# cvlab-epfl/gecco

Measured on NVIDIA B200. Metric: point clouds/sec (2048 pts, full EDM sampler), higher is better.
Workload: dtype bf16

## Files before the change

gecco_b200/csrc/attention_pool_tc.cu:

```cuda
#include "common.cuh"
#include "kernels.cuh"
#include "ptx.cuh"

namespace gecco {
namespace {

constexpr int TM = 128;
constexpr int NI = 64;
constexpr int HD = 48;
constexpr int NH = 8;
constexpr int NP = NH / 2;
constexpr int C = NH * HD;
constexpr int SLOTS = 4;
constexpr int WIN_BYTES = TM * 128;
constexpr int Q_BYTES = 2 * NI * 128;
constexpr int P_BYTES = 2 * TM * 128;
constexpr int TMEM_COLS = 512;
constexpr int THREADS = 128 + 256;
constexpr int SMEM_BYTES = 1024  + 2 * Q_BYTES + 2 * SLOTS * WIN_BYTES + 2 * P_BYTES + 256 ;
static_assert(SMEM_BYTES <= 232448, "shared memory budget");

__host__ __device__ constexpr uint32_t umma_idesc_bf16_bmn(int M, int N) { return umma_idesc_bf16(M, N) | (1u << 16); }
__device__ __forceinline__ uint64_t umma_desc_mn_sw128(uint32_t saddr, uint32_t lbo_bytes) {
  uint64_t d = 0;
  d |= static_cast<uint64_t>((saddr & 0x3FFFFu) >> 4);
  d |= static_cast<uint64_t>(lbo_bytes >> 4) << 16;
  d |= static_cast<uint64_t>(1024 >> 4) << 32;
  d |= static_cast<uint64_t>(1) << 46;
  d |= static_cast<uint64_t>(2) << 61;
  return d;
}

struct PParams {
  const __nv_bfloat16* q_ind;
  int clouds, rows_per_cloud, valid_rows;
  int tiles, splits, tps;
  int items;
  float* partial;
  __nv_bfloat16* out;
  long long ldo;
};

struct Cursor {
  int item, item_stride, items;
  int tile, tile_end;
  int cloud, pair, split;
  __device__ __forceinline__ void open(const PParams& p) {
    if (item >= items) return;
    split = item % p.splits;
    pair = (item / p.splits) % NP;
    cloud = item / (p.splits * NP);
    tile = split * p.tps;
    tile_end = min(p.tiles, tile + p.tps);
  }
  __device__ __forceinline__ void init(const PParams& p, int first, int stride) {
// ... 15 lines not shown
  float y;
  asm("ex2.approx.ftz.f32 %0, %1;" : "=f"(y) : "f"(x));
  return y;
}
__device__ __forceinline__ void tmem_ld32(uint32_t addr, uint32_t (&r)[32]) {
  asm volatile(
      "tcgen05.ld.sync.aligned.32x32b.x32.b32 {%0,%1,%2,%3,%4,%5,%6,%7,%8,%9,%10,%11,%12,%13,%14,%15,%16,%17,%18,%19,%20,"
      "%21,%22,%23,%24,%25,%26,%27,%28,%29,%30,%31}, [%32];"
      : "=r"(r[0]), "=r"(r[1]), "=r"(r[2]), "=r"(r[3]), "=r"(r[4]), "=r"(r[5]), "=r"(r[6]), "=r"(r[7]), "=r"(r[8]),
        "=r"(r[9]), "=r"(r[10]), "=r"(r[11]), "=r"(r[12]), "=r"(r[13]), "=r"(r[14]), "=r"(r[15]), "=r"(r[16]),
        "=r"(r[17]), "=r"(r[18]), "=r"(r[19]), "=r"(r[20]), "=r"(r[21]), "=r"(r[22]), "=r"(r[23]), "=r"(r[24]),
        "=r"(r[25]), "=r"(r[26]), "=r"(r[27]), "=r"(r[28]), "=r"(r[29]), "=r"(r[30]), "=r"(r[31])
      : "r"(addr)
      : "memory");
}
__device__ __forceinline__ void sts128(uint32_t addr, uint32_t a, uint32_t b, uint32_t c, uint32_t d) {
  asm volatile("st.shared.v4.b32 [%0], {%1,%2,%3,%4};" ::"r"(addr), "r"(a), "r"(b), "r"(c), "r"(d) : "memory");
}

__global__ void __launch_bounds__(THREADS, 1)
pool_tc_kernel(const __grid_constant__ CUtensorMap tma_k, const __grid_constant__ CUtensorMap tma_v, const PParams p) {
  extern __shared__ uint8_t smem_raw[];
  uint8_t* smem = reinterpret_cast<uint8_t*>((reinterpret_cast<uintptr_t>(smem_raw) + 1023) & ~uintptr_t(1023));
  uint8_t* sQ = smem;
  uint8_t* sK = sQ + 2 * Q_BYTES;
  uint8_t* sV = sK + SLOTS * WIN_BYTES;
  uint8_t* sP = sV + SLOTS * WIN_BYTES;
  uint64_t* bars = reinterpret_cast<uint64_t*>(sP + 2 * P_BYTES);
  uint64_t* k_full = bars;
  uint64_t* k_empty = k_full + SLOTS;
  uint64_t* v_full = k_empty + SLOTS;
  uint64_t* v_empty = v_full + SLOTS;
  uint64_t* q_ready = v_empty + SLOTS;
  uint64_t* s_full = q_ready + 2;
  uint64_t* p_full = s_full + 2;
  uint64_t* o_full = p_full + 2;
  uint64_t* o_read = o_full + 2;
  uint32_t* tmem_slot = reinterpret_cast<uint32_t*>(o_read + 2);

  const int warp = threadIdx.x >> 5;
  const int uwarp = uniform_warp_idx();
  const int lane = threadIdx.x & 31;

  if (warp == 0 && lane == 0) {
    tma_prefetch_desc(&tma_k);
    tma_prefetch_desc(&tma_v);
  }
  if (warp == 1 && lane == 0) {
    for (int i = 0; i < SLOTS; ++i) {
      mbar_init(&k_full[i], 1);
      mbar_init(&k_empty[i], 1);
      mbar_init(&v_full[i], 1);
      mbar_init(&v_empty[i], 1);
    }
    for (int i = 0; i < 2; ++i) {
      mbar_init(&q_ready[i], 4);
      mbar_init(&s_full[i], 1);
      mbar_init(&p_full[i], 4);
      mbar_init(&o_full[i], 1);
      mbar_init(&o_read[i], 4);
    }
    fence_barrier_init();
  }
  if (warp == 2) tmem_alloc<TMEM_COLS>(tmem_slot);
  tc_fence_before_sync();
  __syncthreads();
  tc_fence_after_sync();
  const uint32_t tmem_base = *tmem_slot;
  pdl_wait();
  pdl_launch_dependents();

  Cursor cur[2];
  cur[0].init(p, blockIdx.x * 2 + 0, gridDim.x * 2);
  cur[1].init(p, blockIdx.x * 2 + 1, gridDim.x * 2);

  if (warp == 0 && lane == 0) {
    uint32_t gk = 0, gv = 0;
    while (!cur[0].done() || !cur[1].done()) {
#pragma unroll
      for (int kind = 0; kind < 2; ++kind) {
#pragma unroll
        for (int w = 0; w < 2; ++w) {
          if (cur[w].done()) continue;
          const int row = cur[w].cloud * p.rows_per_cloud + cur[w].tile * TM;
          for (int j = 0; j < 2; ++j) {
            const int col = kind == 0 ? (2 * cur[w].pair + j) * HD : cur[w].pair * 2 * HD + j * 64;
            if (kind == 0) {
              const uint32_t slot = gk % SLOTS, use = gk / SLOTS;
              mbar_wait(&k_empty[slot], (use & 1u) ^ 1u);
              mbar_arrive_expect_tx(&k_full[slot], WIN_BYTES);
              tma_load_2d(sK + slot * WIN_BYTES, &tma_k, &k_full[slot], col, row);
              ++gk;
            } else {
              const uint32_t slot = gv % SLOTS, use = gv / SLOTS;
              mbar_wait(&v_empty[slot], (use & 1u) ^ 1u);
              mbar_arrive_expect_tx(&v_full[slot], WIN_BYTES);
              tma_load_2d(sV + slot * WIN_BYTES, &tma_v, &v_full[slot], col, row);
              ++gv;
            }
          }
        }
      }
#pragma unroll
      for (int w = 0; w < 2; ++w)
        if (!cur[w].done()) cur[w].next(p);
    }
  } else if (uwarp == 1) {
    constexpr uint32_t idesc_s = umma_idesc_bf16(TM, TM);
    constexpr uint32_t idesc_o = umma_idesc_bf16_bmn(TM, 2 * HD);
    const uint32_t sQ_u = uniform_u32(smem_u32(sQ)), sK_u = uniform_u32(smem_u32(sK)), sV_u = uniform_u32(smem_u32(sV));
    const uint32_t sP_u = uniform_u32(smem_u32(sP));
    const uint32_t tmem_u = uniform_u32(tmem_base);
    uint32_t gk = 0, gv = 0;
    uint32_t nS[2] = {0, 0};
    uint32_t nO[2] = {0, 0};
    uint32_t nQ[2] = {0, 0};
    int pend[2] = {0, 0};
    auto issue_s = [&](int w) {
      if (nS[w] > 0) mbar_wait(&o_read[w], (nS[w] - 1) & 1u);
      if (cur[w].first_of_item(p)) {
        mbar_wait(&q_ready[w], nQ[w] & 1u);
        ++nQ[w];
      }
      const uint32_t k0 = gk % SLOTS, k1 = (gk + 1) % SLOTS;
      mbar_wait(&k_full[k0], (gk / SLOTS) & 1u);
      mbar_wait(&k_full[k1], ((gk + 1) / SLOTS) & 1u);
      tc_fence_after_sync();
      if (elect_one()) {
        const uint32_t qa = sQ_u + w * Q_BYTES;
#pragma unroll
        for (int hh = 0; hh < 2; ++hh) {
          const uint32_t kb = sK_u + (hh ? k1 : k0) * WIN_BYTES;
#pragma unroll
          for (int kk = 0; kk < HD / 16; ++kk)
            umma_bf16_ss(tmem_u + w * 256 + hh * 128, umma_desc_k_sw128(qa) + 2 * kk, umma_desc_k_sw128(kb) + 2 * kk, idesc_s,
                         kk ? 1u : 0u);
        }
        umma_commit(&k_empty[k0]);
        umma_commit(&k_empty[k1]);
        umma_commit(&s_full[w]);
      }
      __syncwarp();
      gk += 2;
      ++nS[w];
      pend[w] = 1;
      cur[w].next(p);
    };
    auto issue_o = [&](int w) {
      mbar_wait(&p_full[w], nO[w] & 1u);
      const uint32_t v0 = gv % SLOTS, v1 = (gv + 1) % SLOTS;
      mbar_wait(&v_full[v0], (gv / SLOTS) & 1u);
      mbar_wait(&v_full[v1], ((gv + 1) / SLOTS) & 1u);
      tc_fence_after_sync();
      if (elect_one()) {
        const uint32_t vb = sV_u + v0 * WIN_BYTES;
#pragma unroll
        for (int kk = 0; kk < TM / 16; ++kk) {
          const uint64_t da = umma_desc_k_sw128(sP_u + w * P_BYTES + (kk >> 2) * (TM * 128)) + 2 * (kk & 3);
          const uint64_t db = umma_desc_mn_sw128(vb + kk * 2048, WIN_BYTES);
          umma_bf16_ss(tmem_u + w * 256, da, db, idesc_o, kk ? 1u : 0u);
        }
        umma_commit(&v_empty[v0]);
        umma_commit(&v_empty[v1]);
        umma_commit(&o_full[w]);
      }
      __syncwarp();
      gv += 2;
      ++nO[w];
      pend[w] = 0;
    };
#pragma unroll
    for (int w = 0; w < 2; ++w)
      if (!cur[w].done()) issue_s(w);
    while (pend[0] || pend[1]) {
#pragma unroll
      for (int w = 0; w < 2; ++w)
        if (pend[w]) issue_o(w);
#pragma unroll
      for (int w = 0; w < 2; ++w)
        if (!cur[w].done()) issue_s(w);
    }
  } else if (warp >= 4) {
    const int w = (warp - 4) >> 2;
    const int q = warp & 3;
    const uint32_t row = q * 32 + lane;
    const uint32_t x7 = (row & 7u) << 4;
    const uint32_t t_addr = tmem_base + (static_cast<uint32_t>(q * 32) << 16) + w * 256 + (q >> 1) * 128;
    const uint32_t o_addr = tmem_base + (static_cast<uint32_t>(q * 32) << 16) + w * 256 + (q >> 1) * HD;
    const uint32_t p_row = smem_u32(sP) + w * P_BYTES + row * 128u;
    Cursor& c = cur[w];
    uint32_t n = 0;
    float m = -INFINITY, l = 0.f;
    float acc[HD];
#pragma unroll
    for (int d = 0; d < HD; ++d) acc[d] = 0.f;

    while (!c.done()) {
      if (c.first_of_item(p)) {
        const int t = threadIdx.x - 128 - w * 128;
        for (int i = t; i < 2 * NI * (HD / 8); i += 128) {
          const int r = i / (HD / 8), ch = i - r * (HD / 8);
          const uint4 v = __ldg(reinterpret_cast<const uint4*>(p.q_ind + ((long long)c.pair * 2 * NI + r) * HD + ch * 8));
          *reinterpret_cast<uint4*>(sQ + w * Q_BYTES + r * 128 + ((ch ^ (r & 7)) << 4)) = v;
        }
        fence_proxy_async_smem();
        __syncwarp();
        if (lane == 0) mbar_arrive(&q_ready[w]);
      }
      const int nvalid = p.valid_rows - c.tile * TM;
      mbar_wait(&s_full[w], n & 1u);
      tc_fence_after_sync();
      float mref = m;
      if (c.first_of_item(p)) {
        float mx = -INFINITY;
#pragma unroll 1
        for (int cb = 0; cb < TM; cb += 32) {
          uint32_t s[32];
          tmem_ld32(t_addr + cb, s);
          tmem_ld_wait();
          if (nvalid >= cb + 32) {
#pragma unroll
            for (int i = 0; i < 32; ++i) mx = fmaxf(mx, __uint_as_float(s[i]));
          } else {
#pragma unroll
            for (int i = 0; i < 32; ++i) mx = fmaxf(mx, cb + i < nvalid ? __uint_as_float(s[i]) : -INFINITY);
          }
        }
        mref = mx;
        m = mx;
      }
      float sum, umax;
      for (;;) {
        sum = 0.f;
        umax = -INFINITY;
#pragma unroll 1
        for (int cb = 0; cb < TM; cb += 32) {
          uint32_t s[32];
          tmem_ld32(t_addr + cb, s);
          tmem_ld_wait();
          uint32_t pk[16];
          if (nvalid >= cb + 32) {
#pragma unroll
            for (int i = 0; i < 16; ++i) {
              const float s0 = __uint_as_float(s[2 * i]), s1 = __uint_as_float(s[2 * i + 1]);
              umax = fmaxf(umax, fmaxf(s0, s1));
              const float a = ex2f(s0 - mref), b = ex2f(s1 - mref);
              sum += a + b;
              pk[i] = pack_bf16x2(a, b);
            }
          } else {
#pragma unroll
            for (int i = 0; i < 16; ++i) {
              const bool v0 = cb + 2 * i < nvalid, v1 = cb + 2 * i + 1 < nvalid;
              const float s0 = v0 ? __uint_as_float(s[2 * i]) : -INFINITY, s1 = v1 ? __uint_as_float(s[2 * i + 1]) : -INFINITY;
              umax = fmaxf(umax, fmaxf(s0, s1));
              const float a = ex2f(s0 - mref), b = ex2f(s1 - mref);
              sum += a + b;
              pk[i] = pack_bf16x2(a, b);
            }
          }
          const uint32_t kb_row = p_row + (cb >> 6) * (TM * 128);
          const uint32_t ch0 = (cb & 32) >> 3;
#pragma unroll
          for (int i = 0; i < 4; ++i)
            sts128(kb_row + (((ch0 + i) << 4) ^ x7), pk[4 * i], pk[4 * i + 1], pk[4 * i + 2], pk[4 * i + 3]);
        }
        if (!__any_sync(0xffffffffu, umax > mref + 64.f)) break;
        if (umax > mref) {
          const float r = ex2f(mref - umax);
          l *= r;
#pragma unroll
          for (int d = 0; d < HD; ++d) acc[d] *= r;
          mref = umax;
          m = umax;
        }
      }
      l += sum;
      fence_proxy_async_smem();
      tc_fence_before_sync();
      __syncwarp();
      if (lane == 0) mbar_arrive(&p_full[w]);
      mbar_wait(&o_full[w], n & 1u);
      tc_fence_after_sync();
      {
        uint32_t o[HD];
        tmem_ld16(o_addr, o);
        tmem_ld16(o_addr + 16, o + 16);
        tmem_ld16(o_addr + 32, o + 32);
        tmem_ld_wait();
        tc_fence_before_sync();
        __syncwarp();
        if (lane == 0) mbar_arrive(&o_read[w]);
#pragma unroll
        for (int d = 0; d < HD; ++d) acc[d] += __uint_as_float(o[d]);
      }
      if (umax > m) {
        const float r = ex2f(m - umax);
        l *= r;
#pragma unroll
        for (int d = 0; d < HD; ++d) acc[d] *= r;
        m = umax;
      }
      ++n;
      if (c.last_of_item()) {
        const int head = 2 * c.pair + (row >> 6), ind = row & 63;
        if (p.splits == 1) {
          const float inv = 1.0f / l;
          uint4* dst = reinterpret_cast<uint4*>(p.out + ((long long)c.cloud * NI + ind) * p.ldo + head * HD);
#pragma unroll
          for (int i = 0; i < HD / 8; ++i)
            dst[i] = make_uint4(pack_bf16x2(acc[8 * i + 0] * inv, acc[8 * i + 1] * inv), pack_bf16x2(acc[8 * i + 2] * inv, acc[8 * i + 3] * inv),
                                pack_bf16x2(acc[8 * i + 4] * inv, acc[8 * i + 5] * inv), pack_bf16x2(acc[8 * i + 6] * inv, acc[8 * i + 7] * inv));
        } else {
          float* dst = p.partial + ((((long long)c.cloud * NH + head) * p.splits + c.split) * NI + ind) * (HD + 2);
#pragma unroll
          for (int d = 0; d < HD; d += 2) *reinterpret_cast<float2*>(dst + d) = make_float2(acc[d], acc[d + 1]);
          *reinterpret_cast<float2*>(dst + HD) = make_float2(m, l);
        }
        m = -INFINITY;
        l = 0.f;
#pragma unroll
        for (int d = 0; d < HD; ++d) acc[d] = 0.f;
      }
      c.next(p);
    }
  }

  tc_fence_before_sync();
  __syncthreads();
  if (warp == 2) {
    tc_fence_after_sync();
    tmem_dealloc<TMEM_COLS>(tmem_base);
  }
}

}

bool pool_tc_supported(const gecco_pool_args& a) {
  return a.heads == NH && a.head_dim == HD && a.inducers == NI && a.rows_per_cloud % TM == 0 && a.ld % 8 == 0 &&
// ... 13 lines not shown
  PParams p;
  p.q_ind = static_cast<const __nv_bfloat16*>(a.q_inducers);
  p.clouds = a.clouds; p.rows_per_cloud = a.rows_per_cloud; p.valid_rows = a.valid_rows;
  p.tiles = ceil_div(a.valid_rows, TM);
  const int sms = sm_count();
  int splits = (2 * sms) / (a.clouds * NP);
  if (splits > a.splits) splits = a.splits;
  if (splits > p.tiles) splits = p.tiles;
  if (splits < 1 || a.partial == nullptr) splits = 1;
  p.tps = ceil_div(p.tiles, splits);
  p.splits = ceil_div(p.tiles, p.tps);
  p.items = a.clouds * NP * p.splits;
  p.partial = a.partial;
  p.out = static_cast<__nv_bfloat16*>(a.out_bf16);
  p.ldo = a.ldo;
  *splits_used = p.splits;
  int grid = ceil_div(p.items, 2);
  if (grid > sms) grid = sms;

  static bool attr_set = false;
  if (!attr_set) {
    cudaError_t e = cudaFuncSetAttribute(pool_tc_kernel, cudaFuncAttributeMaxDynamicSharedMemorySize, SMEM_BYTES);
    if (e != cudaSuccess) return fail_cuda(e, "cudaFuncSetAttribute(pool_tc_kernel)");
    attr_set = true;
  }
  cudaLaunchConfig_t cfg = {};
  cfg.gridDim = dim3(grid);
  cfg.blockDim = dim3(THREADS);
  cfg.dynamicSmemBytes = SMEM_BYTES;
  cfg.stream = stream;
// ... 13 lines not shown
```

gecco_b200/csrc/attention_tc.cu:

```cuda
#include "common.cuh"
#include "kernels.cuh"
#include "ptx.cuh"

namespace gecco {
namespace {

constexpr int TM = 128;
constexpr int NI = 64;
constexpr int HD = 48;
constexpr int NH = 8;
constexpr int C = NH * HD;
constexpr int BK = 64;
constexpr int NKB = C / BK;
constexpr int QSLOTS = 4;
constexpr int Q_SLOT_BYTES = TM * BK * 2;
constexpr int K_KB_BYTES = NI * BK * 2;
constexpr int VT_BYTES = C * NI * 2;
constexpr int P_BYTES = TM * NI * 2;
constexpr int Y_BYTES = TM * HD * 2;
constexpr int O_COLS = C;
constexpr int TMEM_COLS = 512;
constexpr int THREADS = 128 + 256;
constexpr int SMEM_BYTES = 1024  + QSLOTS * Q_SLOT_BYTES + NKB * K_KB_BYTES + VT_BYTES + 2 * P_BYTES + 2 * Y_BYTES +
                           256 ;
static_assert(SMEM_BYTES <= 232448, "shared memory budget");

struct UParams {
  int tiles_per_cloud, num_tiles, tiles_per_cta;
};

__device__ __forceinline__ float ex2f(float x) {
  float y;
  asm("ex2.approx.ftz.f32 %0, %1;" : "=f"(y) : "f"(x));
  return y;
}
__device__ __forceinline__ void tmem_ld32(uint32_t addr, uint32_t (&r)[32]) {
  asm volatile(
      "tcgen05.ld.sync.aligned.32x32b.x32.b32 {%0,%1,%2,%3,%4,%5,%6,%7,%8,%9,%10,%11,%12,%13,%14,%15,%16,%17,%18,%19,%20,"
// ... 5 lines not shown
      : "r"(addr)
      : "memory");
}
__device__ __forceinline__ void sts128(uint32_t addr, uint32_t a, uint32_t b, uint32_t c, uint32_t d) {
  asm volatile("st.shared.v4.b32 [%0], {%1,%2,%3,%4};" ::"r"(addr), "r"(a), "r"(b), "r"(c), "r"(d) : "memory");
}

__global__ void __launch_bounds__(THREADS, 1)
unpool_tc_kernel(const __grid_constant__ CUtensorMap tma_q, const __grid_constant__ CUtensorMap tma_k,
                 const __grid_constant__ CUtensorMap tma_vt, const __grid_constant__ CUtensorMap tma_y, const UParams p) {
  extern __shared__ uint8_t smem_raw[];
  uint8_t* smem = reinterpret_cast<uint8_t*>((reinterpret_cast<uintptr_t>(smem_raw) + 1023) & ~uintptr_t(1023));
  uint8_t* sQ = smem;
  uint8_t* sK = sQ + QSLOTS * Q_SLOT_BYTES;
  uint8_t* sVT = sK + NKB * K_KB_BYTES;
  uint8_t* sP = sVT + VT_BYTES;
  uint8_t* sY = sP + 2 * P_BYTES;
  uint64_t* bars = reinterpret_cast<uint64_t*>(sY + 2 * Y_BYTES);
  uint64_t* q_full = bars;
  uint64_t* q_empty = q_full + QSLOTS;
  uint64_t* kv_full = q_empty + QSLOTS;
  uint64_t* s_full = kv_full + 1;
  uint64_t* p_full = s_full + 2;
  uint64_t* pv_done = p_full + 2;
  uint64_t* tile_done = pv_done + 2;
  uint32_t* tmem_slot = reinterpret_cast<uint32_t*>(tile_done + 1);

  const int warp = threadIdx.x >> 5;
  const int uwarp = uniform_warp_idx();
  const int lane = threadIdx.x & 31;
  const int tile_begin = blockIdx.x * p.tiles_per_cta;
  const int tile_end = min(tile_begin + p.tiles_per_cta, p.num_tiles);

  if (warp == 0 && lane == 0) {
    tma_prefetch_desc(&tma_q);
    tma_prefetch_desc(&tma_k);
    tma_prefetch_desc(&tma_vt);
    tma_prefetch_desc(&tma_y);
  }
  if (warp == 1 && lane == 0) {
    for (int i = 0; i < QSLOTS; ++i) {
      mbar_init(&q_full[i], 1);
      mbar_init(&q_empty[i], 1);
    }
    mbar_init(kv_full, 1);
    mbar_init(tile_done, 1);
    for (int i = 0; i < 2; ++i) {
      mbar_init(&s_full[i], 1);
      mbar_init(&p_full[i], 4);
      mbar_init(&pv_done[i], 1);
    }
    fence_barrier_init();
  }
  if (warp == 2) tmem_alloc<TMEM_COLS>(tmem_slot);
  tc_fence_before_sync();
  __syncthreads();
  tc_fence_after_sync();
  const uint32_t tmem_base = *tmem_slot;
  pdl_wait();
  pdl_launch_dependents();

  if (warp == 0 && lane == 0) {
    int cloud_loaded = -1;
    uint32_t it = 0, g = 0;
    for (int t = tile_begin; t < tile_end; ++t, ++it) {
// ... 5 lines not shown
        tma_load_2d(sVT, &tma_vt, kv_full, 0, cloud * C);
        tma_load_2d(sVT + VT_BYTES / 2, &tma_vt, kv_full, 0, cloud * C + C / 2);
        cloud_loaded = cloud;
      }
      for (int h = 0; h < NH; ++h, ++g) {
        const uint32_t slot = g % QSLOTS, use = g / QSLOTS;
        mbar_wait(&q_empty[slot], (use & 1u) ^ 1u);
        mbar_arrive_expect_tx(&q_full[slot], Q_SLOT_BYTES);
        tma_load_2d(sQ + slot * Q_SLOT_BYTES, &tma_q, &q_full[slot], h * HD, t * TM);
      }
    }
  } else if (uwarp == 1) {
    constexpr uint32_t idesc_s = umma_idesc_bf16(TM, NI);
    constexpr uint32_t idesc_o = umma_idesc_bf16(TM, HD);
    const uint32_t sQ_u = uniform_u32(smem_u32(sQ)), sK_u = uniform_u32(smem_u32(sK));
    const uint32_t sVT_u = uniform_u32(smem_u32(sVT)), sP_u = uniform_u32(smem_u32(sP));
    const uint32_t tmem_u = uniform_u32(tmem_base);
    int cloud_loaded = -1;
    uint32_t it = 0, ncl = 0, gs = 0;
    auto issue_s = [&](int h) {
      const uint32_t slot = gs % QSLOTS, use = gs / QSLOTS;
      mbar_wait(&q_full[slot], use & 1u);
      tc_fence_after_sync();
      if (elect_one()) {
#pragma unroll
        for (int kk = 0; kk < HD / 16; ++kk) {
          const int col = h * HD + kk * 16;
          const uint64_t da = umma_desc_k_sw128(sQ_u + slot * Q_SLOT_BYTES) + 2 * kk;
          const uint64_t db = umma_desc_k_sw128(sK_u + (col / BK) * K_KB_BYTES) + (((col % BK) * 2) >> 4);
          umma_bf16_ss(tmem_u + O_COLS + (h & 1) * NI, da, db, idesc_s, kk ? 1u : 0u);
        }
// ... 8 lines not shown
      if (cloud != cloud_loaded) {
        mbar_wait(kv_full, ncl & 1u);
        tc_fence_after_sync();
        cloud_loaded = cloud;
        ++ncl;
      }
      issue_s(0);
      issue_s(1);
      for (int h = 0; h < NH; ++h) {
        const uint32_t w = h & 1u, use = it * (NH / 2) + (h >> 1);
        mbar_wait(&p_full[w], use & 1u);
        tc_fence_after_sync();
        if (elect_one()) {
#pragma unroll
          for (int kk = 0; kk < NI / 16; ++kk) {
            const uint64_t da = umma_desc_k_sw128(sP_u + w * P_BYTES) + 2 * kk;
            const uint64_t db = umma_desc_k_sw128(sVT_u + h * (HD * 128)) + 2 * kk;
            umma_bf16_ss(tmem_u + h * HD, da, db, idesc_o, kk ? 1u : 0u);
          }
          umma_commit(&pv_done[w]);
        }
        __syncwarp();
        if (h + 2 < NH) issue_s(h + 2);
      }
      if (elect_one()) umma_commit(tile_done);
      __syncwarp();
    }
  } else if (warp >= 4) {
    const int w = (warp - 4) >> 2;
    const int q = warp & 3;
    const uint32_t row = q * 32 + lane;
    const uint32_t x7 = (row & 7u) << 4;
    const uint32_t lane_addr = static_cast<uint32_t>(q * 32) << 16;
    const uint32_t p_row = smem_u32(sP) + w * P_BYTES + row * 128u;
    uint8_t* y_stage = sY + w * Y_BYTES;
    const uint32_t y_row = smem_u32(y_stage) + row * (HD * 2);
    const bool storer = (warp & 3) == 0 && lane == 0;
    uint32_t use = 0;
    float inv_prev = 0.f;
    int t_prev = 0, h_prev = -1;

    auto drain = [&](int t_of, int h_of, float inv) {
      uint32_t o[48];
      tmem_ld16(tmem_base + lane_addr + h_of * HD, o);
      tmem_ld16(tmem_base + lane_addr + h_of * HD + 16, o + 16);
      tmem_ld16(tmem_base + lane_addr + h_of * HD + 32, o + 32);
      tmem_ld_wait();
      tc_fence_before_sync();
      if (storer) tma_store_wait_read<0>();
// ... 28 lines not shown
        for (int i = 0; i < 32; ++i) mx = fmaxf(mx, fmaxf(__uint_as_float(s0[i]), __uint_as_float(s1[i])));
        float sum = 0.f;
        uint32_t pk[32];
#pragma unroll
        for (int i = 0; i < 16; ++i) {
          const float a = ex2f(__uint_as_float(s0[2 * i]) - mx), b = ex2f(__uint_as_float(s0[2 * i + 1]) - mx);
          sum += a + b;
          pk[i] = pack_bf16x2(a, b);
        }
#pragma unroll
        for (int i = 0; i < 16; ++i) {
          const float a = ex2f(__uint_as_float(s1[2 * i]) - mx), b = ex2f(__uint_as_float(s1[2 * i + 1]) - mx);
          sum += a + b;
          pk[16 + i] = pack_bf16x2(a, b);
        }
        if (use > 0) {
          mbar_wait(&pv_done[w], (use - 1) & 1u);
          tc_fence_after_sync();
        }
#pragma unroll
        for (int i = 0; i < 8; ++i) sts128(p_row + ((((uint32_t)i) << 4) ^ x7), pk[4 * i], pk[4 * i + 1], pk[4 * i + 2], pk[4 * i + 3]);
        fence_proxy_async_smem();
        tc_fence_before_sync();
        __syncwarp();
        if (lane == 0) mbar_arrive(&p_full[w]);
        if (h_prev >= 0) drain(t_prev, h_prev, inv_prev);
        inv_prev = 1.0f / sum;
        t_prev = t;
        h_prev = h;
      }
    }
    if (h_prev >= 0) {
      mbar_wait(&pv_done[w], (use - 1) & 1u);
      tc_fence_after_sync();
      drain(t_prev, h_prev, inv_prev);
    }
    if (storer) tma_store_wait_read<0>();
  }

  tc_fence_before_sync();
  __syncthreads();
  if (warp == 2) {
    tc_fence_after_sync();
    tmem_dealloc<TMEM_COLS>(tmem_base);
  }
}

__global__ void __launch_bounds__(256) transpose_v_kernel(const __nv_bfloat16* __restrict__ kv, long long ldkv, int v_off,
// ... 77 lines not shown
```

gecco_b200/csrc/ptx.cuh:

```cuda
#pragma once
#include <cuda.h>
#include <cuda_bf16.h>
#include <cuda_runtime.h>
#include <stdint.h>

#ifdef GECCO_DEBUG_COUNTERS
#define GECCO_DBG_ON(ptr) ((ptr) != nullptr)
#else
#define GECCO_DBG_ON(ptr) (false)
#endif

namespace gecco {

__device__ __forceinline__ uint32_t smem_u32(const void* p) {
  return static_cast<uint32_t>(__cvta_generic_to_shared(p));
}

__device__ __forceinline__ void mbar_init(uint64_t* bar, uint32_t count) {
  asm volatile("mbarrier.init.shared::cta.b64 [%0], %1;" ::"r"(smem_u32(bar)), "r"(count));
}
__device__ __forceinline__ void fence_barrier_init() {
  asm volatile("fence.mbarrier_init.release.cluster;" ::: "memory");
}
__device__ __forceinline__ void mbar_arrive_expect_tx(uint64_t* bar, uint32_t bytes) {
// ... 111 lines not shown
}
template <uint32_t kCols>
__device__ __forceinline__ void tmem_dealloc(uint32_t addr) {
  asm volatile("tcgen05.dealloc.cta_group::1.sync.aligned.b32 %0, %1;" ::"r"(addr), "n"(kCols) : "memory");
}
__device__ __forceinline__ void tmem_ld16(uint32_t addr, uint32_t* r) {
  asm volatile(
      "tcgen05.ld.sync.aligned.32x32b.x16.b32 {%0,%1,%2,%3,%4,%5,%6,%7,%8,%9,%10,%11,%12,%13,%14,%15}, [%16];"
      : "=r"(r[0]), "=r"(r[1]), "=r"(r[2]), "=r"(r[3]), "=r"(r[4]), "=r"(r[5]), "=r"(r[6]), "=r"(r[7]),
        "=r"(r[8]), "=r"(r[9]), "=r"(r[10]), "=r"(r[11]), "=r"(r[12]), "=r"(r[13]), "=r"(r[14]), "=r"(r[15])
      : "r"(addr)
      : "memory");
}
__device__ __forceinline__ void tmem_ld_wait() {
  asm volatile("tcgen05.wait::ld.sync.aligned;" ::: "memory");
}

__device__ __forceinline__ uint64_t umma_desc_k_sw128(uint32_t saddr) {
  uint64_t d = 0;
  d |= static_cast<uint64_t>((saddr & 0x3FFFFu) >> 4);
  d |= static_cast<uint64_t>(1) << 16;
  d |= static_cast<uint64_t>(1024 >> 4) << 32;
  d |= static_cast<uint64_t>(1) << 46;
  d |= static_cast<uint64_t>(2) << 61;
  return d;
}
__host__ __device__ constexpr uint32_t umma_idesc_bf16(int M, int N) {
  return (1u << 4) | (1u << 7) | (1u << 10) | (static_cast<uint32_t>(N >> 3) << 17) |
         (static_cast<uint32_t>(M >> 4) << 24);
}
__device__ __forceinline__ void umma_bf16_ss(uint32_t tmem_d, uint64_t desc_a, uint64_t desc_b, uint32_t idesc,
                                             uint32_t accumulate) {
  asm volatile(
      "{\n\t.reg .pred p;\n\t"
      "setp.ne.b32 p, %4, 0;\n\t"
      "tcgen05.mma.cta_group::1.kind::f16 [%0], %1, %2, %3, p;\n\t}"
      ::"r"(tmem_d), "l"(desc_a), "l"(desc_b), "r"(idesc), "r"(accumulate)
      : "memory");
}
__device__ __forceinline__ void umma_commit(uint64_t* bar) {
  asm volatile("tcgen05.commit.cta_group::1.mbarrier::arrive::one.shared::cluster.b64 [%0];" ::"r"(smem_u32(bar))
               : "memory");
}

constexpr uint32_t kPeerBitMask = 0xFEFFFFFFu;
__device__ __forceinline__ uint32_t cluster_ctarank() {
  uint32_t r;
  asm volatile("mov.u32 %0, %%cluster_ctarank;" : "=r"(r));
  return r;
}
__device__ __forceinline__ void cluster_sync_all() {
  asm volatile("barrier.cluster.arrive.release.aligned;" ::: "memory");
  asm volatile("barrier.cluster.wait.acquire.aligned;" ::: "memory");
}
// ... 76 lines not shown
```

gecco_b200/csrc/umma_bench.cu:

```cuda
#include "common.cuh"
#include "debug_api.h"
#include "ptx.cuh"

namespace gecco {
namespace {

__device__ __forceinline__ uint64_t desc_sw128(uint32_t saddr, uint32_t lbo_bytes) {
  uint64_t d = 0;
  d |= static_cast<uint64_t>((saddr & 0x3FFFFu) >> 4);
  d |= static_cast<uint64_t>(lbo_bytes >> 4) << 16;
  d |= static_cast<uint64_t>(1024 >> 4) << 32;
  d |= static_cast<uint64_t>(1) << 46;
  d |= static_cast<uint64_t>(2) << 61;
  return d;
}
__device__ __forceinline__ void umma_bf16_ts(uint32_t tmem_d, uint32_t tmem_a, uint64_t desc_b, uint32_t idesc, uint32_t accumulate) {
  asm volatile(
      "{\n\t.reg .pred p;\n\t"
      "setp.ne.b32 p, %4, 0;\n\t"
      "tcgen05.mma.cta_group::1.kind::f16 [%0], [%1], %2, %3, p;\n\t}"
      ::"r"(tmem_d), "r"(tmem_a), "l"(desc_b), "r"(idesc), "r"(accumulate)
      : "memory");
}

constexpr int UB_SMEM = 1024 + 16384  + 65536  + 64;

__global__ void __launch_bounds__(128, 1) umma_bench_kernel(int mode, int n, int batch, int reps, long long* out) {
  extern __shared__ uint8_t smem_raw[];
  uint8_t* smem = reinterpret_cast<uint8_t*>((reinterpret_cast<uintptr_t>(smem_raw) + 1023) & ~uintptr_t(1023));
  uint8_t* sA = smem;
  uint8_t* sB = sA + 16384;
  uint64_t* bar = reinterpret_cast<uint64_t*>(sB + 65536);
  uint32_t* tmem_slot = reinterpret_cast<uint32_t*>(bar + 1);
  for (int i = threadIdx.x; i < (16384 + 65536) / 16; i += blockDim.x) reinterpret_cast<uint4*>(smem)[i] = make_uint4(0, 0, 0, 0);
  const int warp = threadIdx.x >> 5, lane = threadIdx.x & 31;
  if (warp == 0 && lane == 0) {
    mbar_init(bar, 1);
// ... 71 lines not shown
```

Measured before the change: 119.2.

## Keep softmax P in TMEM and accumulate O in tensor memory for attention kernels

```diff
diff --git a/gecco_b200/csrc/attention_pool_tc.cu b/gecco_b200/csrc/attention_pool_tc.cu
--- a/gecco_b200/csrc/attention_pool_tc.cu
+++ b/gecco_b200/csrc/attention_pool_tc.cu
@@ -3,6 +3,7 @@
 #include "ptx.cuh"
 
 namespace gecco {
+extern long long* g_gemm_debug;
 namespace {
 
 constexpr int TM = 128;
@@ -11,14 +12,16 @@
 constexpr int NH = 8;
 constexpr int NP = NH / 2;
 constexpr int C = NH * HD;
-constexpr int SLOTS = 4;
-constexpr int WIN_BYTES = TM * 128;
-constexpr int Q_BYTES = 2 * NI * 128;
-constexpr int P_BYTES = 2 * TM * 128;
+constexpr int KSLOTS = 5;
+constexpr int VSLOTS = 6;
+constexpr int BOX_BYTES = TM * 128;
+constexpr int A_BYTES = 3 * NI * 128;
+constexpr int O_COL = 128;
 constexpr int TMEM_COLS = 512;
 constexpr int THREADS = 128 + 256;
-constexpr int SMEM_BYTES = 1024  + 2 * Q_BYTES + 2 * SLOTS * WIN_BYTES + 2 * P_BYTES + 256 ;
+constexpr int SMEM_BYTES = 1024  + 2 * A_BYTES + (KSLOTS + VSLOTS) * BOX_BYTES + 256 ;
 static_assert(SMEM_BYTES <= 232448, "shared memory budget");
+static_assert(VSLOTS % 2 == 0, "the two V boxes of a unit must be adjacent: the second is the B operand's next atom");
 
 __host__ __device__ constexpr uint32_t umma_idesc_bf16_bmn(int M, int N) { return umma_idesc_bf16(M, N) | (1u << 16); }
 __device__ __forceinline__ uint64_t umma_desc_mn_sw128(uint32_t saddr, uint32_t lbo_bytes) {
@@ -39,6 +42,7 @@
   float* partial;
   __nv_bfloat16* out;
   long long ldo;
+  long long* dbg;
 };
 
 struct Cursor {
@@ -84,29 +88,36 @@
       : "r"(addr)
       : "memory");
 }
-__device__ __forceinline__ void sts128(uint32_t addr, uint32_t a, uint32_t b, uint32_t c, uint32_t d) {
-  asm volatile("st.shared.v4.b32 [%0], {%1,%2,%3,%4};" ::"r"(addr), "r"(a), "r"(b), "r"(c), "r"(d) : "memory");
+__device__ __forceinline__ void rescale_o(uint32_t o_addr, float r) {
+  uint32_t o[HD];
+  tmem_ld16(o_addr, o);
+  tmem_ld16(o_addr + 16, o + 16);
+  tmem_ld16(o_addr + 32, o + 32);
+  tmem_ld_wait();
+#pragma unroll
+  for (int d = 0; d < HD; ++d) o[d] = __float_as_uint(__uint_as_float(o[d]) * r);
+  tmem_st16(o_addr, o);
+  tmem_st16(o_addr + 16, o + 16);
+  tmem_st16(o_addr + 32, o + 32);
 }
 
 __global__ void __launch_bounds__(THREADS, 1)
 pool_tc_kernel(const __grid_constant__ CUtensorMap tma_k, const __grid_constant__ CUtensorMap tma_v, const PParams p) {
   extern __shared__ uint8_t smem_raw[];
   uint8_t* smem = reinterpret_cast<uint8_t*>((reinterpret_cast<uintptr_t>(smem_raw) + 1023) & ~uintptr_t(1023));
-  uint8_t* sQ = smem;
-  uint8_t* sK = sQ + 2 * Q_BYTES;
-  uint8_t* sV = sK + SLOTS * WIN_BYTES;
-  uint8_t* sP = sV + SLOTS * WIN_BYTES;
-  uint64_t* bars = reinterpret_cast<uint64_t*>(sP + 2 * P_BYTES);
+  uint8_t* sA = smem;
+  uint8_t* sK = sA + 2 * A_BYTES;
+  uint8_t* sV = sK + KSLOTS * BOX_BYTES;
+  uint64_t* bars = reinterpret_cast<uint64_t*>(sV + VSLOTS * BOX_BYTES);
   uint64_t* k_full = bars;
-  uint64_t* k_empty = k_full + SLOTS;
-  uint64_t* v_full = k_empty + SLOTS;
-  uint64_t* v_empty = v_full + SLOTS;
-  uint64_t* q_ready = v_empty + SLOTS;
+  uint64_t* k_empty = k_full + KSLOTS;
+  uint64_t* v_full = k_empty + KSLOTS;
+  uint64_t* v_empty = v_full + VSLOTS;
+  uint64_t* q_ready = v_empty + VSLOTS;
   uint64_t* s_full = q_ready + 2;
   uint64_t* p_full = s_full + 2;
   uint64_t* o_full = p_full + 2;
-  uint64_t* o_read = o_full + 2;
-  uint32_t* tmem_slot = reinterpret_cast<uint32_t*>(o_read + 2);
+  uint32_t* tmem_slot = reinterpret_cast<uint32_t*>(o_full + 2);
 
   const int warp = threadIdx.x >> 5;
   const int uwarp = uniform_warp_idx();
@@ -117,9 +128,11 @@
     tma_prefetch_desc(&tma_v);
   }
   if (warp == 1 && lane == 0) {
-    for (int i = 0; i < SLOTS; ++i) {
+    for (int i = 0; i < KSLOTS; ++i) {
       mbar_init(&k_full[i], 1);
       mbar_init(&k_empty[i], 1);
+    }
+    for (int i = 0; i < VSLOTS; ++i) {
       mbar_init(&v_full[i], 1);
       mbar_init(&v_empty[i], 1);
     }
@@ -128,7 +141,6 @@
       mbar_init(&s_full[i], 1);
       mbar_init(&p_full[i], 4);
       mbar_init(&o_full[i], 1);
-      mbar_init(&o_read[i], 4);
     }
     fence_barrier_init();
   }
@@ -154,18 +166,18 @@
           if (cur[w].done()) continue;
           const int row = cur[w].cloud * p.rows_per_cloud + cur[w].tile * TM;
           for (int j = 0; j < 2; ++j) {
-            const int col = kind == 0 ? (2 * cur[w].pair + j) * HD : cur[w].pair * 2 * HD + j * 64;
+            const int col = cur[w].pair * 2 * HD + j * 64;
             if (kind == 0) {
-              const uint32_t slot = gk % SLOTS, use = gk / SLOTS;
+              const uint32_t slot = gk % KSLOTS, use = gk / KSLOTS;
               mbar_wait(&k_empty[slot], (use & 1u) ^ 1u);
-              mbar_arrive_expect_tx(&k_full[slot], WIN_BYTES);
-              tma_load_2d(sK + slot * WIN_BYTES, &tma_k, &k_full[slot], col, row);
+              mbar_arrive_expect_tx(&k_full[slot], BOX_BYTES);
+              tma_load_2d(sK + slot * BOX_BYTES, &tma_k, &k_full[slot], col, row);
               ++gk;
             } else {
-              const uint32_t slot = gv % SLOTS, use = gv / SLOTS;
+              const uint32_t slot = gv % VSLOTS, use = gv / VSLOTS;
               mbar_wait(&v_empty[slot], (use & 1u) ^ 1u);
-              mbar_arrive_expect_tx(&v_full[slot], WIN_BYTES);
-              tma_load_2d(sV + slot * WIN_BYTES, &tma_v, &v_full[slot], col, row);
+              mbar_arrive_expect_tx(&v_full[slot], BOX_BYTES);
+              tma_load_2d(sV + slot * BOX_BYTES, &tma_v, &v_full[slot], col, row);
               ++gv;
             }
           }
@@ -178,33 +190,34 @@
   } else if (uwarp == 1) {
     constexpr uint32_t idesc_s = umma_idesc_bf16(TM, TM);
     constexpr uint32_t idesc_o = umma_idesc_bf16_bmn(TM, 2 * HD);
-    const uint32_t sQ_u = uniform_u32(smem_u32(sQ)), sK_u = uniform_u32(smem_u32(sK)), sV_u = uniform_u32(smem_u32(sV));
-    const uint32_t sP_u = uniform_u32(smem_u32(sP));
+    const uint32_t sA_u = uniform_u32(smem_u32(sA)), sK_u = uniform_u32(smem_u32(sK)), sV_u = uniform_u32(smem_u32(sV));
     const uint32_t tmem_u = uniform_u32(tmem_base);
     uint32_t gk = 0, gv = 0;
-    uint32_t nS[2] = {0, 0};
-    uint32_t nO[2] = {0, 0};
+    uint32_t nP[2] = {0, 0};
     uint32_t nQ[2] = {0, 0};
     int pend[2] = {0, 0};
+    int pfirst[2] = {0, 0}, plast[2] = {0, 0};
+    long long c_s = 0, c_o = 0, c_t0 = 0;
+    if (GECCO_DBG_ON(p.dbg)) c_t0 = clock64();
     auto issue_s = [&](int w) {
-      if (nS[w] > 0) mbar_wait(&o_read[w], (nS[w] - 1) & 1u);
-      if (cur[w].first_of_item(p)) {
+      long long t0 = 0;
+      if (GECCO_DBG_ON(p.dbg)) t0 = clock64();
+      const bool first = cur[w].first_of_item(p);
+      if (first) {
         mbar_wait(&q_ready[w], nQ[w] & 1u);
         ++nQ[w];
       }
-      const uint32_t k0 = gk % SLOTS, k1 = (gk + 1) % SLOTS;
-      mbar_wait(&k_full[k0], (gk / SLOTS) & 1u);
-      mbar_wait(&k_full[k1], ((gk + 1) / SLOTS) & 1u);
+      const uint32_t k0 = gk % KSLOTS, k1 = (gk + 1) % KSLOTS;
+      mbar_wait(&k_full[k0], (gk / KSLOTS) & 1u);
+      mbar_wait(&k_full[k1], ((gk + 1) / KSLOTS) & 1u);
       tc_fence_after_sync();
       if (elect_one()) {
-        const uint32_t qa = sQ_u + w * Q_BYTES;
-#pragma unroll
-        for (int hh = 0; hh < 2; ++hh) {
-          const uint32_t kb = sK_u + (hh ? k1 : k0) * WIN_BYTES;
-#pragma unroll
-          for (int kk = 0; kk < HD / 16; ++kk)
-            umma_bf16_ss(tmem_u + w * 256 + hh * 128, umma_desc_k_sw128(qa) + 2 * kk, umma_desc_k_sw128(kb) + 2 * kk, idesc_s,
-                         kk ? 1u : 0u);
+        const uint32_t a = sA_u + w * A_BYTES;
+#pragma unroll
+        for (int j = 0; j < 6; ++j) {
+          const uint64_t da = umma_desc_k_sw128(a + (j < 3 ? 0 : NI * 128)) + 2 * (j % 3);
+          const uint64_t db = umma_desc_k_sw128(sK_u + (j < 4 ? k0 : k1) * BOX_BYTES) + 2 * (j & 3);
+          umma_bf16_ss(tmem_u + w * 256, da, db, idesc_s, j ? 1u : 0u);
         }
         umma_commit(&k_empty[k0]);
         umma_commit(&k_empty[k1]);
@@ -212,81 +225,101 @@
       }
       __syncwarp();
       gk += 2;
-      ++nS[w];
       pend[w] = 1;
+      pfirst[w] = first;
+      plast[w] = cur[w].last_of_item();
       cur[w].next(p);
+      if (GECCO_DBG_ON(p.dbg)) c_s += clock64() - t0;
     };
     auto issue_o = [&](int w) {
-      mbar_wait(&p_full[w], nO[w] & 1u);
-      const uint32_t v0 = gv % SLOTS, v1 = (gv + 1) % SLOTS;
-      mbar_wait(&v_full[v0], (gv / SLOTS) & 1u);
-      mbar_wait(&v_full[v1], ((gv + 1) / SLOTS) & 1u);
+      long long t0 = 0;
+      if (GECCO_DBG_ON(p.dbg)) t0 = clock64();
+      mbar_wait(&p_full[w], nP[w] & 1u);
+      const uint32_t v0 = gv % VSLOTS, v1 = v0 + 1;
+      mbar_wait(&v_full[v0], (gv / VSLOTS) & 1u);
+      mbar_wait(&v_full[v1], (gv / VSLOTS) & 1u);
       tc_fence_after_sync();
       if (elect_one()) {
-        const uint32_t vb = sV_u + v0 * WIN_BYTES;
+        const uint32_t vb = sV_u + v0 * BOX_BYTES;
 #pragma unroll
         for (int kk = 0; kk < TM / 16; ++kk) {
-          const uint64_t da = umma_desc_k_sw128(sP_u + w * P_BYTES + (kk >> 2) * (TM * 128)) + 2 * (kk & 3);
-          const uint64_t db = umma_desc_mn_sw128(vb + kk * 2048, WIN_BYTES);
-          umma_bf16_ss(tmem_u + w * 256, da, db, idesc_o, kk ? 1u : 0u);
+          const uint64_t db = umma_desc_mn_sw128(vb + kk * 2048, BOX_BYTES);
+          umma_bf16_ts(tmem_u + w * 256 + O_COL, tmem_u + w * 256 + kk * 8, db, idesc_o, (pfirst[w] && kk == 0) ? 0u : 1u);
         }
         umma_commit(&v_empty[v0]);
         umma_commit(&v_empty[v1]);
-        umma_commit(&o_full[w]);
+        if (plast[w]) umma_commit(&o_full[w]);
       }
       __syncwarp();
       gv += 2;
-      ++nO[w];
+      ++nP[w];
       pend[w] = 0;
+      if (GECCO_DBG_ON(p.dbg)) c_o += clock64() - t0;
     };
 #pragma unroll
     for (int w = 0; w < 2; ++w)
       if (!cur[w].done()) issue_s(w);
     while (pend[0] || pend[1]) {
 #pragma unroll
-      for (int w = 0; w < 2; ++w)
-        if (pend[w]) issue_o(w);
-#pragma unroll
-      for (int w = 0; w < 2; ++w)
+      for (int w = 0; w < 2; ++w) {
+        if (!pend[w]) continue;
+        issue_o(w);
         if (!cur[w].done()) issue_s(w);
+      }
+    }
+    if (GECCO_DBG_ON(p.dbg) && lane == 0) {
+      long long* d = p.dbg + (long long)blockIdx.x * 32 + 16;
+      d[0] = c_s;
+      d[1] = c_o;
+      d[2] = clock64() - c_t0;
     }
   } else if (warp >= 4) {
     const int w = (warp - 4) >> 2;
     const int q = warp & 3;
     const uint32_t row = q * 32 + lane;
-    const uint32_t x7 = (row & 7u) << 4;
-    const uint32_t t_addr = tmem_base + (static_cast<uint32_t>(q * 32) << 16) + w * 256 + (q >> 1) * 128;
-    const uint32_t o_addr = tmem_base + (static_cast<uint32_t>(q * 32) << 16) + w * 256 + (q >> 1) * HD;
-    const uint32_t p_row = smem_u32(sP) + w * P_BYTES + row * 128u;
+    const uint32_t s_addr = tmem_base + (static_cast<uint32_t>(q * 32) << 16) + w * 256;
+    const uint32_t o_addr = s_addr + O_COL + (q >> 1) * HD;
+    const int t = threadIdx.x - 128 - w * 128;
+    uint8_t* sAw = sA + w * A_BYTES;
+    for (int i = t; i < NI * 128 / 16; i += 128) reinterpret_cast<uint4*>(sAw + NI * 128)[i] = make_uint4(0, 0, 0, 0);
     Cursor& c = cur[w];
-    uint32_t n = 0;
+    uint32_t n = 0, items_done = 0;
     float m = -INFINITY, l = 0.f;
-    float acc[HD];
-#pragma unroll
-    for (int d = 0; d < HD; ++d) acc[d] = 0.f;
+    float rpend = 1.f;
+    long long c_ws = 0, c_sm = 0, c_wo = 0, c_or = 0, c_t0 = 0, tc = 0;
+    if (GECCO_DBG_ON(p.dbg)) c_t0 = clock64();
 
     while (!c.done()) {
-      if (c.first_of_item(p)) {
-        const int t = threadIdx.x - 128 - w * 128;
+      const bool first = c.first_of_item(p);
+      if (first) {
         for (int i = t; i < 2 * NI * (HD / 8); i += 128) {
           const int r = i / (HD / 8), ch = i - r * (HD / 8);
+          const int br = r < NI ? r : r + NI;
           const uint4 v = __ldg(reinterpret_cast<const uint4*>(p.q_ind + ((long long)c.pair * 2 * NI + r) * HD + ch * 8));
-          *reinterpret_cast<uint4*>(sQ + w * Q_BYTES + r * 128 + ((ch ^ (r & 7)) << 4)) = v;
+          *reinterpret_cast<uint4*>(sAw + br * 128 + ((ch ^ (br & 7)) << 4)) = v;
         }
         fence_proxy_async_smem();
         __syncwarp();
         if (lane == 0) mbar_arrive(&q_ready[w]);
       }
       const int nvalid = p.valid_rows - c.tile * TM;
+      if (GECCO_DBG_ON(p.dbg)) tc = clock64();
       mbar_wait(&s_full[w], n & 1u);
+      if (GECCO_DBG_ON(p.dbg)) {
+        const long long t = clock64();
+        c_ws += t - tc;
+        tc = t;
+      }
       tc_fence_after_sync();
+      if (!first && __any_sync(0xffffffffu, rpend != 1.f)) rescale_o(o_addr, rpend);
+      rpend = 1.f;
       float mref = m;
-      if (c.first_of_item(p)) {
+      if (first) {
         float mx = -INFINITY;
 #pragma unroll 1
         for (int cb = 0; cb < TM; cb += 32) {
           uint32_t s[32];
-          tmem_ld32(t_addr + cb, s);
+          tmem_ld32(s_addr + cb, s);
           tmem_ld_wait();
           if (nvalid >= cb + 32) {
 #pragma unroll
@@ -300,15 +333,15 @@
         m = mx;
       }
       float sum, umax;
+      uint32_t pk[TM / 2];
       for (;;) {
         sum = 0.f;
         umax = -INFINITY;
-#pragma unroll 1
+#pragma unroll
         for (int cb = 0; cb < TM; cb += 32) {
           uint32_t s[32];
-          tmem_ld32(t_addr + cb, s);
+          tmem_ld32(s_addr + cb, s);
           tmem_ld_wait();
-          uint32_t pk[16];
           if (nvalid >= cb + 32) {
 #pragma unroll
             for (int i = 0; i < 16; ++i) {
@@ -316,7 +349,7 @@
               umax = fmaxf(umax, fmaxf(s0, s1));
               const float a = ex2f(s0 - mref), b = ex2f(s1 - mref);
               sum += a + b;
-              pk[i] = pack_bf16x2(a, b);
+              pk[cb / 2 + i] = pack_bf16x2(a, b);
             }
           } else {
 #pragma unroll
@@ -326,53 +359,53 @@
               umax = fmaxf(umax, fmaxf(s0, s1));
               const float a = ex2f(s0 - mref), b = ex2f(s1 - mref);
               sum += a + b;
-              pk[i] = pack_bf16x2(a, b);
+              pk[cb / 2 + i] = pack_bf16x2(a, b);
             }
           }
-          const uint32_t kb_row = p_row + (cb >> 6) * (TM * 128);
-          const uint32_t ch0 = (cb & 32) >> 3;
-#pragma unroll
-          for (int i = 0; i < 4; ++i)
-            sts128(kb_row + (((ch0 + i) << 4) ^ x7), pk[4 * i], pk[4 * i + 1], pk[4 * i + 2], pk[4 * i + 3]);
         }
         if (!__any_sync(0xffffffffu, umax > mref + 64.f)) break;
+        const float r = umax > mref ? ex2f(mref - umax) : 1.f;
+        l *= r;
+        if (!first) rescale_o(o_addr, r);
         if (umax > mref) {
-          const float r = ex2f(mref - umax);
-          l *= r;
-#pragma unroll
-          for (int d = 0; d < HD; ++d) acc[d] *= r;
           mref = umax;
           m = umax;
         }
       }
       l += sum;
-      fence_proxy_async_smem();
+#pragma unroll
+      for (int i = 0; i < TM / 2; i += 16) tmem_st16(s_addr + i, pk + i);
+      tmem_st_wait();
       tc_fence_before_sync();
       __syncwarp();
       if (lane == 0) mbar_arrive(&p_full[w]);
-      mbar_wait(&o_full[w], n & 1u);
-      tc_fence_after_sync();
-      {
+      if (GECCO_DBG_ON(p.dbg)) c_sm += clock64() - tc;
+      if (umax > m) {
+        const float r = ex2f(m - umax);
+        l *= r;
+        rpend = r;
+        m = umax;
+      }
+      ++n;
+      if (c.last_of_item()) {
+        if (GECCO_DBG_ON(p.dbg)) tc = clock64();
+        mbar_wait(&o_full[w], items_done & 1u);
+        if (GECCO_DBG_ON(p.dbg)) {
+          const long long t = clock64();
+          c_wo += t - tc;
+          tc = t;
+        }
+        ++items_done;
+        tc_fence_after_sync();
         uint32_t o[HD];
         tmem_ld16(o_addr, o);
         tmem_ld16(o_addr + 16, o + 16);
         tmem_ld16(o_addr + 32, o + 32);
         tmem_ld_wait();
         tc_fence_before_sync();
-        __syncwarp();
-        if (lane == 0) mbar_arrive(&o_read[w]);
-#pragma unroll
-        for (int d = 0; d < HD; ++d) acc[d] += __uint_as_float(o[d]);
-      }
-      if (umax > m) {
-        const float r = ex2f(m - umax);
-        l *= r;
-#pragma unroll
-        for (int d = 0; d < HD; ++d) acc[d] *= r;
-        m = umax;
-      }
-      ++n;
-      if (c.last_of_item()) {
+        float acc[HD];
+#pragma unroll
+        for (int d = 0; d < HD; ++d) acc[d] = __uint_as_float(o[d]) * rpend;
         const int head = 2 * c.pair + (row >> 6), ind = row & 63;
         if (p.splits == 1) {
           const float inv = 1.0f / l;
@@ -389,10 +422,19 @@
         }
         m = -INFINITY;
         l = 0.f;
-#pragma unroll
-        for (int d = 0; d < HD; ++d) acc[d] = 0.f;
+        rpend = 1.f;
+        if (GECCO_DBG_ON(p.dbg)) c_or += clock64() - tc;
       }
       c.next(p);
+    }
+    if (GECCO_DBG_ON(p.dbg) && t == 0) {
+      long long* d = p.dbg + (long long)blockIdx.x * 32 + w * 8;
+      d[0] = c_ws;
+      d[1] = c_sm;
+      d[2] = c_wo;
+      d[3] = c_or;
+      d[4] = clock64() - c_t0;
+      d[5] = n;
     }
   }
 
@@ -436,6 +478,7 @@
   p.partial = a.partial;
   p.out = static_cast<__nv_bfloat16*>(a.out_bf16);
   p.ldo = a.ldo;
+  p.dbg = g_gemm_debug;
   *splits_used = p.splits;
   int grid = ceil_div(p.items, 2);
   if (grid > sms) grid = sms;
diff --git a/gecco_b200/csrc/attention_tc.cu b/gecco_b200/csrc/attention_tc.cu
--- a/gecco_b200/csrc/attention_tc.cu
+++ b/gecco_b200/csrc/attention_tc.cu
@@ -12,16 +12,15 @@
 constexpr int C = NH * HD;
 constexpr int BK = 64;
 constexpr int NKB = C / BK;
-constexpr int QSLOTS = 4;
+constexpr int QSLOTS = 6;
 constexpr int Q_SLOT_BYTES = TM * BK * 2;
 constexpr int K_KB_BYTES = NI * BK * 2;
 constexpr int VT_BYTES = C * NI * 2;
-constexpr int P_BYTES = TM * NI * 2;
 constexpr int Y_BYTES = TM * HD * 2;
 constexpr int O_COLS = C;
 constexpr int TMEM_COLS = 512;
 constexpr int THREADS = 128 + 256;
-constexpr int SMEM_BYTES = 1024  + QSLOTS * Q_SLOT_BYTES + NKB * K_KB_BYTES + VT_BYTES + 2 * P_BYTES + 2 * Y_BYTES +
+constexpr int SMEM_BYTES = 1024  + QSLOTS * Q_SLOT_BYTES + NKB * K_KB_BYTES + VT_BYTES + 2 * Y_BYTES +
                            256 ;
 static_assert(SMEM_BYTES <= 232448, "shared memory budget");
 
@@ -57,16 +56,14 @@
   uint8_t* sQ = smem;
   uint8_t* sK = sQ + QSLOTS * Q_SLOT_BYTES;
   uint8_t* sVT = sK + NKB * K_KB_BYTES;
-  uint8_t* sP = sVT + VT_BYTES;
-  uint8_t* sY = sP + 2 * P_BYTES;
+  uint8_t* sY = sVT + VT_BYTES;
   uint64_t* bars = reinterpret_cast<uint64_t*>(sY + 2 * Y_BYTES);
   uint64_t* q_full = bars;
   uint64_t* q_empty = q_full + QSLOTS;
   uint64_t* kv_full = q_empty + QSLOTS;
   uint64_t* s_full = kv_full + 1;
   uint64_t* p_full = s_full + 2;
-  uint64_t* pv_done = p_full + 2;
-  uint64_t* tile_done = pv_done + 2;
+  uint64_t* tile_done = p_full + 2;
   uint32_t* tmem_slot = reinterpret_cast<uint32_t*>(tile_done + 1);
 
   const int warp = threadIdx.x >> 5;
@@ -91,7 +88,6 @@
     for (int i = 0; i < 2; ++i) {
       mbar_init(&s_full[i], 1);
       mbar_init(&p_full[i], 4);
-      mbar_init(&pv_done[i], 1);
     }
     fence_barrier_init();
   }
@@ -127,7 +123,7 @@
     constexpr uint32_t idesc_s = umma_idesc_bf16(TM, NI);
     constexpr uint32_t idesc_o = umma_idesc_bf16(TM, HD);
     const uint32_t sQ_u = uniform_u32(smem_u32(sQ)), sK_u = uniform_u32(smem_u32(sK));
-    const uint32_t sVT_u = uniform_u32(smem_u32(sVT)), sP_u = uniform_u32(smem_u32(sP));
+    const uint32_t sVT_u = uniform_u32(smem_u32(sVT));
     const uint32_t tmem_u = uniform_u32(tmem_base);
     int cloud_loaded = -1;
     uint32_t it = 0, ncl = 0, gs = 0;
@@ -166,11 +162,9 @@
         if (elect_one()) {
 #pragma unroll
           for (int kk = 0; kk < NI / 16; ++kk) {
-            const uint64_t da = umma_desc_k_sw128(sP_u + w * P_BYTES) + 2 * kk;
             const uint64_t db = umma_desc_k_sw128(sVT_u + h * (HD * 128)) + 2 * kk;
-            umma_bf16_ss(tmem_u + h * HD, da, db, idesc_o, kk ? 1u : 0u);
+            umma_bf16_ts(tmem_u + h * HD, tmem_u + O_COLS + w * NI + kk * 8, db, idesc_o, kk ? 1u : 0u);
           }
-          umma_commit(&pv_done[w]);
         }
         __syncwarp();
         if (h + 2 < NH) issue_s(h + 2);
@@ -182,9 +176,7 @@
     const int w = (warp - 4) >> 2;
     const int q = warp & 3;
     const uint32_t row = q * 32 + lane;
-    const uint32_t x7 = (row & 7u) << 4;
     const uint32_t lane_addr = static_cast<uint32_t>(q * 32) << 16;
-    const uint32_t p_row = smem_u32(sP) + w * P_BYTES + row * 128u;
     uint8_t* y_stage = sY + w * Y_BYTES;
     const uint32_t y_row = smem_u32(y_stage) + row * (HD * 2);
     const bool storer = (warp & 3) == 0 && lane == 0;
@@ -243,13 +235,9 @@
           sum += a + b;
           pk[16 + i] = pack_bf16x2(a, b);
         }
-        if (use > 0) {
-          mbar_wait(&pv_done[w], (use - 1) & 1u);
-          tc_fence_after_sync();
-        }
-#pragma unroll
-        for (int i = 0; i < 8; ++i) sts128(p_row + ((((uint32_t)i) << 4) ^ x7), pk[4 * i], pk[4 * i + 1], pk[4 * i + 2], pk[4 * i + 3]);
-        fence_proxy_async_smem();
+        tmem_st16(tmem_base + lane_addr + O_COLS + w * NI, pk);
+        tmem_st16(tmem_base + lane_addr + O_COLS + w * NI + 16, pk + 16);
+        tmem_st_wait();
         tc_fence_before_sync();
         __syncwarp();
         if (lane == 0) mbar_arrive(&p_full[w]);
@@ -260,7 +248,7 @@
       }
     }
     if (h_prev >= 0) {
-      mbar_wait(&pv_done[w], (use - 1) & 1u);
+      mbar_wait(tile_done, (tile_end - tile_begin - 1) & 1u);
       tc_fence_after_sync();
       drain(t_prev, h_prev, inv_prev);
     }
diff --git a/gecco_b200/csrc/ptx.cuh b/gecco_b200/csrc/ptx.cuh
--- a/gecco_b200/csrc/ptx.cuh
+++ b/gecco_b200/csrc/ptx.cuh
@@ -149,6 +149,16 @@
 }
 __device__ __forceinline__ void tmem_ld_wait() {
   asm volatile("tcgen05.wait::ld.sync.aligned;" ::: "memory");
+}
+__device__ __forceinline__ void tmem_st16(uint32_t addr, const uint32_t* r) {
+  asm volatile(
+      "tcgen05.st.sync.aligned.32x32b.x16.b32 [%0], {%1,%2,%3,%4,%5,%6,%7,%8,%9,%10,%11,%12,%13,%14,%15,%16};"
+      ::"r"(addr), "r"(r[0]), "r"(r[1]), "r"(r[2]), "r"(r[3]), "r"(r[4]), "r"(r[5]), "r"(r[6]), "r"(r[7]), "r"(r[8]),
+        "r"(r[9]), "r"(r[10]), "r"(r[11]), "r"(r[12]), "r"(r[13]), "r"(r[14]), "r"(r[15])
+      : "memory");
+}
+__device__ __forceinline__ void tmem_st_wait() {
+  asm volatile("tcgen05.wait::st.sync.aligned;" ::: "memory");
 }
 
 __device__ __forceinline__ uint64_t umma_desc_k_sw128(uint32_t saddr) {
@@ -173,6 +183,15 @@
       ::"r"(tmem_d), "l"(desc_a), "l"(desc_b), "r"(idesc), "r"(accumulate)
       : "memory");
 }
+__device__ __forceinline__ void umma_bf16_ts(uint32_t tmem_d, uint32_t tmem_a, uint64_t desc_b, uint32_t idesc,
+                                             uint32_t accumulate) {
+  asm volatile(
+      "{\n\t.reg .pred p;\n\t"
+      "setp.ne.b32 p, %4, 0;\n\t"
+      "tcgen05.mma.cta_group::1.kind::f16 [%0], [%1], %2, %3, p;\n\t}"
+      ::"r"(tmem_d), "r"(tmem_a), "l"(desc_b), "r"(idesc), "r"(accumulate)
+      : "memory");
+}
 __device__ __forceinline__ void umma_commit(uint64_t* bar) {
   asm volatile("tcgen05.commit.cta_group::1.mbarrier::arrive::one.shared::cluster.b64 [%0];" ::"r"(smem_u32(bar))
                : "memory");
diff --git a/gecco_b200/csrc/umma_bench.cu b/gecco_b200/csrc/umma_bench.cu
--- a/gecco_b200/csrc/umma_bench.cu
+++ b/gecco_b200/csrc/umma_bench.cu
@@ -13,14 +13,6 @@
   d |= static_cast<uint64_t>(1) << 46;
   d |= static_cast<uint64_t>(2) << 61;
   return d;
-}
-__device__ __forceinline__ void umma_bf16_ts(uint32_t tmem_d, uint32_t tmem_a, uint64_t desc_b, uint32_t idesc, uint32_t accumulate) {
-  asm volatile(
-      "{\n\t.reg .pred p;\n\t"
-      "setp.ne.b32 p, %4, 0;\n\t"
-      "tcgen05.mma.cta_group::1.kind::f16 [%0], [%1], %2, %3, p;\n\t}"
-      ::"r"(tmem_d), "r"(tmem_a), "l"(desc_b), "r"(idesc), "r"(accumulate)
-      : "memory");
 }
 
 constexpr int UB_SMEM = 1024 + 16384  + 65536  + 64;
```

Result: faster. 121.4, median of 6 (+1.8%).
